# LeCAR-Lab/CoVO-MPC

Hardware: AMD Instinct MI355X
Metric: mpc_control_steps_per_sec (higher is better)
Workload: dtype f32; 1 GPU; covo-online tracking_zigzag N=65536 H=32 lam=0.01 sigma=0.5 (teacher-forced on the recorded inputs -- noisy state, a_mean, key -- of this controller's own 300-step closed-loop episode, timed steps spread evenly over the episode; samples sharded 1x65536, one exchange of the 516-float rank records per step: collective); controller=covo-online, task=tracking_zigzag, N_global=65536, N_local=65536, H=32, pos_stats_info=False

## Files before the change

covo_mpc_amd/csrc/hessian_adj_body.hpp:

```cpp
constexpr int NX = ADJ_NX, NZ = NX + 4, NH = NX + 1, HH = COVO_H, NA = COVO_NA;
constexpr size_t WS_X = 0;
constexpr size_t WS_JF = WS_X + 32 * 16;
constexpr size_t WS_GL = WS_JF + 32 * NX * NZ;
constexpr size_t WS_LAM = WS_GL + 32 * 16;
constexpr size_t WS_MXX = WS_LAM + 33 * 16;
constexpr size_t WS_MXU = WS_MXX + 32 * 256;
constexpr size_t WS_MUU = WS_MXU + 32 * 64;
constexpr size_t WS_S = WS_MUU + 32 * 16;
constexpr int NPAIR = NZ * (NZ + 1) / 2;
constexpr int PAIR_THREADS = (NPAIR + 63) / 64 * 64;
constexpr size_t WS_COUNT = WS_S + (size_t)32 * 16 * NA + 2;
constexpr unsigned long long ADJ_LAM_UNSET = 0xFFF7ADEADBEEF000ull;


__device__ __forceinline__ void adj_force(const float *__restrict__ st, const AdjArgs &A, int bi, int k, double (&f)[3])
{
    if (k == 0) {
        f[0] = st[ST_FDIST + 0]; f[1] = st[ST_FDIST + 1]; f[2] = st[ST_FDIST + 2];
    } else if (A.f_tab != nullptr) {
        const float4 r = A.f_tab[(size_t)bi * HH + k];
        f[0] = r.x; f[1] = r.y; f[2] = r.z;
    } else {
        f[0] = f[1] = f[2] = 0.0;
    }
}

__device__ __forceinline__ void adj_targets(const float *__restrict__ st, const float *__restrict__ pos_traj,
                                            const float *__restrict__ vel_traj, int T, int time0, int k, double (&tar)[6])
{
    if (k == 0) {
        for (int i = 0; i < 3; ++i) { tar[i] = st[ST_POSTAR + i]; tar[3 + i] = st[ST_VELTAR + i]; }
    } else {
        int idx = time0 + k;
        idx = idx < 0 ? 0 : (idx > T - 1 ? T - 1 : idx);
        for (int i = 0; i < 3; ++i) { tar[i] = pos_traj[3 * idx + i]; tar[3 + i] = vel_traj[3 * idx + i]; }
    }
}

#define ADJ_FOR_STATE(OP) OP(px, 0) OP(py, 1) OP(pz, 2) OP(vx, 3) OP(vy, 4) OP(vz, 5) OP(qx, 6) OP(qy, 7) OP(qz, 8) OP(qw, 9) OP(ox, 10) OP(oy, 11) OP(oz, 12)

__device__ __forceinline__ void adj_store_state(const qm::State<double> &p, double *__restrict__ x)
{
#define OP(m, i) x[i] = p.m;
    ADJ_FOR_STATE(OP)
#undef OP
}
__device__ __forceinline__ void adj_load_state(qm::State<double> &p, const double *__restrict__ x)
{
#define OP(m, i) p.m = x[i];
    ADJ_FOR_STATE(OP)
#undef OP
}

#if ADJ_FS
struct AdjDrag {
    double k, off[3];
};
__device__ __forceinline__ AdjDrag adj_drag(const AdjArgs &A, int bi)
{
    AdjDrag D = {A.drag_k, {A.drag_off[0], A.drag_off[1], A.drag_off[2]}};
    if (A.models != nullptr) {
        const dm::Model m = A.models[bi];
        D.k = adj_drag_coeff(m);
        for (int i = 0; i < 3; ++i) D.off[i] = 0.5 * (double)m.dp[i];
    }
    return D;
}
template <class S>
__device__ __forceinline__ void adj_next_force(const AdjArgs &A, const AdjDrag &D, int bi, int k, const qm::State<S> &s, const S (&f)[3],
                                               S (&fn)[3])
{
    if (k + 1 >= HH) {
        fn[0] = fn[1] = fn[2] = S{};
        return;
    }
    const float4 r = A.f_tab[(size_t)bi * HH + k + 1];
    const double g[3] = {r.x, r.y, r.z}, c = r.w;
    const S v[3] = {s.vx, s.vy, s.vz};
#pragma unroll
    for (int i = 0; i < 3; ++i) fn[i] = (f[i] * c + g[i]) + qm::drag_force<S, double>(v[i], D.off[i], D.k);
}
#endif


#if !ADJ_FS
struct AdjQuat {
    double x, y, z, w;
};
__device__ __forceinline__ AdjQuat adj_qmul(const AdjQuat &a, const AdjQuat &b)
{
    AdjQuat r;
    r.x = fma(a.w, b.x, fma(a.x, b.w, fma(a.y, b.z, -(a.z * b.y))));
    r.y = fma(a.w, b.y, fma(a.y, b.w, fma(a.z, b.x, -(a.x * b.z))));
    r.z = fma(a.w, b.z, fma(a.z, b.w, fma(a.x, b.y, -(a.y * b.x))));
    r.w = fma(a.w, b.w, -fma(a.x, b.x, fma(a.y, b.y, a.z * b.z)));
    return r;
}
template <int CTRL>
__device__ __forceinline__ AdjQuat adj_qdpp(const AdjQuat &q)
{
    return AdjQuat{wr::dpp_f64<CTRL>(q.x), wr::dpp_f64<CTRL>(q.y), wr::dpp_f64<CTRL>(q.z), wr::dpp_f64<CTRL>(q.w)};
}
__device__ __forceinline__ double adj_scan_sum(double v, const double (&pw)[4], double pr, int lane)
{
    v = fma(wr::dpp_f64<0x111>(v), pw[0], v);
    v = fma(wr::dpp_f64<0x112>(v), pw[1], v);
    v = fma(wr::dpp_f64<0x114>(v), pw[2], v);
    v = fma(wr::dpp_f64<0x118>(v), pw[3], v);
    const double t = wr::dpp_f64<0x142>(v);
    return ((lane & 16) != 0) ? fma(t, pr, v) : v;
}
template <bool FT>
__device__ __forceinline__ qm::State<double> adj_prefix_scan(const qm::State<double> &p0, const double (*sact)[4], const double (*sfd)[3],
                                                             const qm::Consts<double> &c, int lane)
{
    const int k = lane & 31, lo = lane & 15;
    const double one[4] = {1.0, 1.0, 1.0, 1.0};
    double pa[4];
    pa[0] = c.alpha;
    pa[1] = pa[0] * pa[0];
    pa[2] = pa[1] * pa[1];
    pa[3] = pa[2] * pa[2];
    const double a16 = pa[3] * pa[3];
    double alo = 1.0;
    if (lo & 1) alo *= pa[0];
    if (lo & 2) alo *= pa[1];
    if (lo & 4) alo *= pa[2];
    if (lo & 8) alo *= pa[3];
    const double ak = (k & 16) ? alo * a16 : alo, apr = alo * c.alpha;
    const double th = sact[k][0];
    double cx = sact[k][1] * c.one_m_alpha, cy = sact[k][2] * c.one_m_alpha, cz = sact[k][3] * c.one_m_alpha;
    cx = adj_scan_sum(cx, pa, apr, lane);
    cy = adj_scan_sum(cy, pa, apr, lane);
    cz = adj_scan_sum(cz, pa, apr, lane);
    const double ox = fma(ak, p0.ox, wr::dpp_f64<0x138>(cx));
    const double oy = fma(ak, p0.oy, wr::dpp_f64<0x138>(cy));
    const double oz = fma(ak, p0.oz, wr::dpp_f64<0x138>(cz));
    AdjQuat P{ox * c.half_dt, oy * c.half_dt, oz * c.half_dt, 1.0};
    {
        AdjQuat t = adj_qdpp<0x111>(P);
        if (lo >= 1) P = adj_qmul(t, P);
        t = adj_qdpp<0x112>(P);
        if (lo >= 2) P = adj_qmul(t, P);
        t = adj_qdpp<0x114>(P);
        if (lo >= 4) P = adj_qmul(t, P);
        t = adj_qdpp<0x118>(P);
        if (lo >= 8) P = adj_qmul(t, P);
        t = adj_qdpp<0x142>(P);
        if (lane & 16) P = adj_qmul(t, P);
    }
    AdjQuat E = adj_qdpp<0x138>(P);
    if (lane == 0) E = AdjQuat{0.0, 0.0, 0.0, 1.0};
    AdjQuat q0{p0.qx, p0.qy, p0.qz, p0.qw};
    {
        const double rn = qm::rsq64_(fma(q0.x, q0.x, fma(q0.y, q0.y, fma(q0.z, q0.z, q0.w * q0.w))));
        q0.x *= rn; q0.y *= rn; q0.z *= rn; q0.w *= rn;
    }
    AdjQuat q = adj_qmul(q0, E);
    if (k > 0) {
        const double rn = qm::rsq64_(fma(q.x, q.x, fma(q.y, q.y, fma(q.z, q.z, q.w * q.w))));
        q.x *= rn; q.y *= rn; q.z *= rn; q.w *= rn;
    }
    const double fx = (FT || k == 0) ? sfd[k][0] : 0.0, fy = (FT || k == 0) ? sfd[k][1] : 0.0, fz = (FT || k == 0) ? sfd[k][2] : 0.0;
    const double Qz0 = 2.0 * (q.x * q.z + q.y * q.w), Qz1 = 2.0 * (q.y * q.z - q.x * q.w), Qz2 = q.w * q.w - q.x * q.x - q.y * q.y + q.z * q.z;
    double dvx = ((Qz0 * th + fx) * c.inv_m) * c.dt, dvy = ((Qz1 * th + fy) * c.inv_m) * c.dt, dvz = ((Qz2 * th + fz) * c.inv_m + c.neg_g) * c.dt;
    dvx = adj_scan_sum(dvx, one, 1.0, lane);
    dvy = adj_scan_sum(dvy, one, 1.0, lane);
    dvz = adj_scan_sum(dvz, one, 1.0, lane);
    const double vx = p0.vx + wr::dpp_f64<0x138>(dvx), vy = p0.vy + wr::dpp_f64<0x138>(dvy), vz = p0.vz + wr::dpp_f64<0x138>(dvz);
    double dpx = adj_scan_sum(vx * c.dt, one, 1.0, lane), dpy = adj_scan_sum(vy * c.dt, one, 1.0, lane), dpz = adj_scan_sum(vz * c.dt, one, 1.0, lane);
    qm::State<double> r;
    r.px = p0.px + wr::dpp_f64<0x138>(dpx);
    r.py = p0.py + wr::dpp_f64<0x138>(dpy);
    r.pz = p0.pz + wr::dpp_f64<0x138>(dpz);
    r.vx = vx; r.vy = vy; r.vz = vz;
    r.qx = (k == 0) ? p0.qx : q.x; r.qy = (k == 0) ? p0.qy : q.y; r.qz = (k == 0) ? p0.qz : q.z; r.qw = (k == 0) ? p0.qw : q.w;
    r.ox = ox; r.oy = oy; r.oz = oz;
    return r;
}
#endif

__device__ __forceinline__ void adj_hd_step(const float *__restrict__ st, const float *__restrict__ am, const AdjArgs &A, int bi,
                                            int time0, int k, const qm::State<double> &p, int a, int b, qm::HD &r,
                                            qm::State<qm::HD> &s
#if ADJ_FS
                                            , const double (&pf)[3], qm::HD (&fn)[3]
#endif
)
{
    const qm::Consts<double> c = A.cs ? A.cs[bi] : A.c;
#define OP(m, i) s.m = qm::HD{p.m, a == i ? 1.0 : 0.0, b == i ? 1.0 : 0.0, 0.0};
    ADJ_FOR_STATE(OP)
#undef OP
#if ADJ_FS
    qm::HD fh[3];
#pragma unroll
    for (int i = 0; i < 3; ++i) {
        fh[i] = qm::HD{pf[i], a == 13 + i ? 1.0 : 0.0, b == 13 + i ? 1.0 : 0.0, 0.0};
        fn[i] = fh[i];
    }
#endif
    r = qm::hd(0.0);
    if (k >= 1) {
        double tar[6];
        adj_targets(st, A.pos_traj + bi * A.traj_stride, A.vel_traj + bi * A.traj_stride, A.T, time0, k, tar);
        r = qm::reward_kind<qm::HD, double>(A.reward, s, tar[0], tar[1], tar[2], tar[3], tar[4], tar[5]);
    }
    if (k <= HH - 2) {
        qm::HD act[4];
#pragma unroll
        for (int d = 0; d < 4; ++d) {
            const qm::HD x{(double)am[4 * k + d], a == NX + d ? 1.0 : 0.0, b == NX + d ? 1.0 : 0.0, 0.0};
            act[d] = qm::clip11_(qm::clip11_(x));
        }
#if ADJ_FS
        adj_next_force<qm::HD>(A, adj_drag(A, bi), bi, k, s, fh, fn);
        qm::dyn_step<qm::HD, double, true, qm::HD>(s, act[0], act[1], act[2], act[3], c, fh[0], fh[1], fh[2]);
#else
        double f[3];
        adj_force(st, A, bi, k, f);
        qm::dyn_step<qm::HD, double>(s, act[0], act[1], act[2], act[3], c, f[0], f[1], f[2]);
#endif
    }
}

template <bool FT>
__global__ __launch_bounds__(64) void adj_jac_kernel(const AdjArgs A)
{
    const int k = blockIdx.x, b = blockIdx.y, lane = threadIdx.x;
    const float *__restrict__ st = A.state + (size_t)b * COVO_STATE_FLOATS;
    const bool raw = A.a_mean_raw != nullptr;
    const float *__restrict__ am_base = raw ? A.a_mean_raw : A.a_mean + (size_t)b * NA;
    const bool shift = raw && A.begin_pass == 0;
    auto am = [&](int i) { return am_base[(shift && i < NA - 4) ? i + 4 : i]; };
    if (raw && k == 0) {
        float *shift_out = const_cast<float *>(A.a_mean);
        shift_out[lane] = am(lane);
        shift_out[lane + 64] = am(lane + 64);
        if (lane < 4) {
            if (A.begin_pass > 0) {
                const uint32_t p0 = A.dyn_out[10], p1 = A.dyn_out[11];
                uint32_t rk[2];
                step_begin_derive_next(lane, p0, p1, A.shared_noise_scale, A.dyn_out, rk);
            } else {
                step_begin_derive(lane, A.blk, A.derive_keys, A.shared_noise_scale, A.dyn_out);
            }
        }
        if (lane == 4 && A.seq != nullptr) A.seq[0] = A.seq[0] + 1u;
    }
    double *__restrict__ ws = A.ws + (size_t)b * WS_COUNT;
    if (lane < 16) {
        reinterpret_cast<unsigned long long *>(ws + WS_LAM)[16 * k + lane] = ADJ_LAM_UNSET;
        if (k == HH - 1) reinterpret_cast<unsigned long long *>(ws + WS_LAM)[16 * HH + lane] = ADJ_LAM_UNSET;
    }
    const int time0 = __float_as_int(st[ST_TIME]);
    const qm::Consts<double> c = A.cs ? A.cs[b] : A.c;
    qm::State<double> p;
    p.px = st[ST_POS + 0]; p.py = st[ST_POS + 1]; p.pz = st[ST_POS + 2];
    p.vx = st[ST_VEL + 0]; p.vy = st[ST_VEL + 1]; p.vz = st[ST_VEL + 2];
    p.qx = st[ST_QUAT + 0]; p.qy = st[ST_QUAT + 1]; p.qz = st[ST_QUAT + 2]; p.qw = st[ST_QUAT + 3];
    p.ox = st[ST_OMEGA + 0]; p.oy = st[ST_OMEGA + 1]; p.oz = st[ST_OMEGA + 2];
    __shared__ double sact[HH][4];
    __shared__ double sfd[HH][3];
    if (lane < HH) {
        double f[3];
        adj_force(st, A, b, lane, f);
        sfd[lane][0] = f[0]; sfd[lane][1] = f[1]; sfd[lane][2] = f[2];
    }
    if (lane < HH) {
        const double a0 = qm::clip11_((double)am(4 * lane + 0)), a1 = qm::clip11_((double)am(4 * lane + 1));
        const double a2 = qm::clip11_((double)am(4 * lane + 2)), a3 = qm::clip11_((double)am(4 * lane + 3));
        sact[lane][0] = (a0 + 1.0) * c.thrust_half;
        sact[lane][1] = a1 * c.komega[0];
        sact[lane][2] = a2 * c.komega[1];
        sact[lane][3] = a3 * c.komega[2];
    }
    __syncthreads();
#if ADJ_FS
    const AdjDrag D = adj_drag(A, b);
    double pf[3] = {sfd[0][0], sfd[0][1], sfd[0][2]};
    for (int t = 0; t < k; ++t) {
        const double th = sact[t][0], w0 = sact[t][1], w1 = sact[t][2], w2 = sact[t][3];
        double fn[3];
        adj_next_force<double>(A, D, b, t, p, pf, fn);
        if (t == 0) qm::dyn_core<double, double>(p, th, w0, w1, w2, c, pf[0], pf[1], pf[2]);
        else qm::dyn_core<double, double, false>(p, th, w0, w1, w2, c, pf[0], pf[1], pf[2]);
        pf[0] = fn[0]; pf[1] = fn[1]; pf[2] = fn[2];
    }
    if (lane == 0) {
        adj_store_state(p, ws + WS_X + 16 * k);
        ws[WS_X + 16 * k + 13] = pf[0]; ws[WS_X + 16 * k + 14] = pf[1]; ws[WS_X + 16 * k + 15] = pf[2];
    }
#else
    if (A.scan_prefix) {
        const qm::State<double> ps = adj_prefix_scan<FT>(p, sact, sfd, c, lane);
#define OP(m, i) p.m = wr::bcast_lane(ps.m, k);
        ADJ_FOR_STATE(OP)
#undef OP
    } else {
        for (int t = 0; t < k; ++t) {
            const double th = sact[t][0], w0 = sact[t][1], w1 = sact[t][2], w2 = sact[t][3];
            if (t == 0) qm::dyn_core<double, double>(p, th, w0, w1, w2, c, sfd[0][0], sfd[0][1], sfd[0][2]);
            else if (FT) qm::dyn_core<double, double, false>(p, th, w0, w1, w2, c, sfd[t][0], sfd[t][1], sfd[t][2]);
            else qm::dyn_core<double, double, false>(p, th, w0, w1, w2, c, 0.0, 0.0, 0.0);
        }
    }
    if (lane == 0) adj_store_state(p, ws + WS_X + 16 * k);
#endif
    qm::State<qm::D1> s;
#define OP(m, i) s.m = qm::D1{p.m, lane == i ? 1.0 : 0.0};
    ADJ_FOR_STATE(OP)
#undef OP
#if ADJ_FS
    qm::D1 fd[3], fdn[3];
#pragma unroll
    for (int i = 0; i < 3; ++i) {
        fd[i] = qm::D1{pf[i], lane == 13 + i ? 1.0 : 0.0};
        fdn[i] = fd[i];
    }
#endif
    qm::D1 r{0.0, 0.0};
    if (k >= 1) {
        double tar[6];
        adj_targets(st, A.pos_traj + b * A.traj_stride, A.vel_traj + b * A.traj_stride, A.T, time0, k, tar);
        r = qm::reward_kind<qm::D1, double>(A.reward, s, tar[0], tar[1], tar[2], tar[3], tar[4], tar[5]);
    }
    if (k <= HH - 2) {
        qm::D1 act[4];
#pragma unroll
        for (int d = 0; d < 4; ++d) {
            const qm::D1 x{(double)am(4 * k + d), lane == NX + d ? 1.0 : 0.0};
            act[d] = qm::clip11_(qm::clip11_(x));
        }
#if ADJ_FS
        adj_next_force<qm::D1>(A, D, b, k, s, fd, fdn);
        qm::dyn_step<qm::D1, double, true, qm::D1>(s, act[0], act[1], act[2], act[3], c, fd[0], fd[1], fd[2]);
#else
        qm::dyn_step<qm::D1, double>(s, act[0], act[1], act[2], act[3], c, sfd[k][0], sfd[k][1], sfd[k][2]);
#endif
    }
    if (lane < NZ) {
        if (lane < NX) ws[WS_GL + 16 * k + lane] = r.a;
        if (k <= HH - 2) {
            double *__restrict__ jf = ws + WS_JF + (size_t)k * NX * NZ;
#define OP(m, i) jf[i * NZ + lane] = s.m.a;
            ADJ_FOR_STATE(OP)
#undef OP
#if ADJ_FS
            jf[13 * NZ + lane] = fdn[0].a; jf[14 * NZ + lane] = fdn[1].a; jf[15 * NZ + lane] = fdn[2].a;
#endif
        }
    }
}

__device__ __forceinline__ void adj_hd_pairs(const AdjArgs &A, int k, int b, int tid)
{
    if (tid >= NPAIR) return;
    const float *__restrict__ st = A.state + (size_t)b * COVO_STATE_FLOATS;
    const float *__restrict__ am = A.a_mean + (size_t)b * NA;
    double *__restrict__ ws = A.ws + (size_t)b * WS_COUNT;
    const int time0 = __float_as_int(st[ST_TIME]);
    int q = tid, a = 0;
    while (q >= NZ - a) { q -= NZ - a; ++a; }
    const int bb = a + q;
    qm::State<double> p;
    adj_load_state(p, ws + WS_X + 16 * k);
    qm::HD r;
    qm::State<qm::HD> s;
#if ADJ_FS
    const double pf[3] = {ws[WS_X + 16 * k + 13], ws[WS_X + 16 * k + 14], ws[WS_X + 16 * k + 15]};
    qm::HD fn[3];
    adj_hd_step(st, am, A, b, time0, k, p, a, bb, r, s, pf, fn);
#else
    adj_hd_step(st, am, A, b, time0, k, p, a, bb, r, s);
#endif
    double h[NH];
    h[0] = r.ab;
#define OP(m, i) h[1 + i] = s.m.ab;
    ADJ_FOR_STATE(OP)
#undef OP
#if ADJ_FS
    h[14] = fn[0].ab; h[15] = fn[1].ab; h[16] = fn[2].ab;
#endif
    double g = h[0];
    if (k <= HH - 2) {
        const double *__restrict__ Lk = ws + WS_LAM + 16 * (k + 1);
        double lam[NX];
        const long long t0 = wall_clock64();
        for (;;) {
            bool unset = false;
#pragma unroll
            for (int i = 0; i < NX; ++i) {
                lam[i] = __hip_atomic_load(Lk + i, __ATOMIC_RELAXED, __HIP_MEMORY_SCOPE_AGENT);
                unset |= (unsigned long long)__double_as_longlong(lam[i]) == ADJ_LAM_UNSET;
            }
            if (!unset) break;
            if (wall_clock64() - t0 > 50000000LL) {
                if (A.status != nullptr) __hip_atomic_fetch_or(A.status, COVO_DEVSTAT_ADJOINT, __ATOMIC_RELAXED, __HIP_MEMORY_SCOPE_SYSTEM);
                break;
            }
            __builtin_amdgcn_s_sleep(2);
        }
#pragma unroll
        for (int i = 0; i < NX; ++i) g = fma(lam[i], h[1 + i], g);
    }
    double *__restrict__ Mxx = ws + WS_MXX + (size_t)k * 256, *__restrict__ Mxu = ws + WS_MXU + (size_t)k * 64;
    double *__restrict__ Muu = ws + WS_MUU + (size_t)k * 16;
    if (bb < NX) {
        Mxx[a * 16 + bb] = g;
        Mxx[bb * 16 + a] = g;
    } else if (a < NX) {
        Mxu[a * 4 + (bb - NX)] = g;
    } else {
        Muu[(a - NX) * 4 + (bb - NX)] = g;
        Muu[(bb - NX) * 4 + (a - NX)] = g;
    }
}

__device__ __forceinline__ void adj_hd_padding(const AdjArgs &A, int k, int b, int tid, int nthreads)
{
    double *__restrict__ ws = A.ws + (size_t)b * WS_COUNT;
    double *__restrict__ Mxx = ws + WS_MXX + (size_t)k * 256, *__restrict__ Mxu = ws + WS_MXU + (size_t)k * 64;
    for (int e = tid; e < 256; e += nthreads)
        if ((e >> 4) >= NX || (e & 15) >= NX) Mxx[e] = 0.0;
    if (tid < (16 - NX) * 4) Mxu[NX * 4 + tid] = 0.0;
}

__global__ __launch_bounds__(256) void adj_hd_kernel(const AdjArgs A)
{
    adj_hd_padding(A, (int)blockIdx.x, (int)blockIdx.y, (int)threadIdx.x, 256);
    adj_hd_pairs(A, (int)blockIdx.x, (int)blockIdx.y, (int)threadIdx.x);
}

__global__ __launch_bounds__(256) void adj_chain_kernel(const AdjArgs A)
{
    __shared__ double sjf[(HH - 1) * NX * NZ + 1];
    __shared__ double sgl[HH * 16];
    const int b = blockIdx.y, tid = threadIdx.x, lane = tid & 63, lo = lane & 15, hi = lane >> 4;
    const int w = blockIdx.x;
    double *__restrict__ ws = A.ws + (size_t)b * WS_COUNT;
#ifdef KC_STAMPS
    const long long kc0 = wall_clock64();
#endif
    if (w >= 9) {
        adj_hd_padding(A, w - 9, b, tid, 256);
        adj_hd_pairs(A, w - 9, b, tid);
        return;
    }
    {
        constexpr int NJ = (HH - 1) * NX * NZ, TJ = (NJ + 255) / 256;
        double vj[TJ];
#pragma unroll
        for (int t = 0; t < TJ; ++t) vj[t] = (tid + 256 * t < NJ) ? ws[WS_JF + tid + 256 * t] : 0.0;
        const double vg0 = ws[WS_GL + tid], vg1 = ws[WS_GL + 256 + tid];
#pragma unroll
        for (int t = 0; t < TJ; ++t)
            if (tid + 256 * t < NJ) sjf[tid + 256 * t] = vj[t];
        sgl[tid] = vg0;
        sgl[256 + tid] = vg1;
        if (tid == 0) sjf[NJ] = 0.0;
    }
#ifdef KC_STAMPS
    const long long kc1 = wall_clock64();
#endif
    __syncthreads();
#ifdef KC_STAMPS
    const long long kc2 = wall_clock64();
#define KC_STAMP_END()                                                                                                       \
    do {                                                                                                                     \
        if (tid == 0 && b == 0 && (w == 0 || w == 7 || w == 8))                                                              \
            printf("KC wg %d: filled %lld first-mfma %lld end %lld (10 ns ticks from entry)\n", w, kc1 - kc0, kc2 - kc0,      \
                   (long long)wall_clock64() - kc0);                                                                         \
    } while (0)
#else
#define KC_STAMP_END() do { } while (0)
#endif
    if (tid >= 64) return;
    constexpr int ZI = (HH - 1) * NX * NZ;
    if (w == 8) {
        const double *__restrict__ G = sgl;
        double *__restrict__ L = ws + WS_LAM;
        f64x4 lam;
#pragma unroll
        for (int r = 0; r < 4; ++r) lam[r] = (lo == 0 && hi + 4 * r < NX) ? G[16 * (HH - 1) + hi + 4 * r] : 0.0;
        if (lo == 0) {
#pragma unroll
            for (int r = 0; r < 4; ++r) {
                __hip_atomic_store(&L[16 * (HH - 1) + hi + 4 * r], lam[r], __ATOMIC_RELAXED, __HIP_MEMORY_SCOPE_AGENT);
                __hip_atomic_store(&L[16 * HH + hi + 4 * r], 0.0, __ATOMIC_RELAXED, __HIP_MEMORY_SCOPE_AGENT);
            }
        }
        int offA[4];
        bool okA[4];
#pragma unroll
        for (int g = 0; g < 4; ++g) {
            okA[g] = lo < NX && 4 * g + hi < NX;
            offA[g] = (4 * g + hi) * NZ + lo;
        }
        bool okG[4];
#pragma unroll
        for (int r = 0; r < 4; ++r) okG[r] = lo == 0 && hi + 4 * r < NX;
        double an[4];
        f64x4 gn;
#pragma unroll
        for (int g = 0; g < 4; ++g) an[g] = sjf[okA[g] ? (HH - 2) * NX * NZ + offA[g] : ZI];
#pragma unroll
        for (int r = 0; r < 4; ++r) gn[r] = okG[r] ? G[16 * (HH - 2) + hi + 4 * r] : 0.0;
#pragma unroll
        for (int k = HH - 2; k >= 1; --k) {
            double ac[4];
            f64x4 acc = gn;
#pragma unroll
            for (int g = 0; g < 4; ++g) ac[g] = an[g];
            if (k > 1) {
#pragma unroll
                for (int g = 0; g < 4; ++g) an[g] = sjf[okA[g] ? (k - 1) * NX * NZ + offA[g] : ZI];
#pragma unroll
                for (int r = 0; r < 4; ++r) gn[r] = okG[r] ? G[16 * (k - 1) + hi + 4 * r] : 0.0;
            }
#pragma unroll
            for (int g = 0; g < 4; ++g) acc = __builtin_amdgcn_mfma_f64_16x16x4f64(ac[g], lam[g], acc, 0, 0, 0);
            lam = acc;
            if (lo == 0) {
#pragma unroll
                for (int r = 0; r < 4; ++r) __hip_atomic_store(&L[16 * k + hi + 4 * r], lam[r], __ATOMIC_RELAXED, __HIP_MEMORY_SCOPE_AGENT);
            }
        }
        KC_STAMP_END();
        return;
    }
    const int col = 16 * w + lo, tcol = col >> 2, dcol = col & 3, k0 = 4 * w;
    double *__restrict__ S = ws + WS_S;
    for (int k = 0; k <= k0; ++k) {
#pragma unroll
        for (int r = 0; r < 4; ++r) S[((size_t)k * 16 + hi + 4 * r) * NA + col] = 0.0;
    }
    f64x4 sv = {0.0, 0.0, 0.0, 0.0};
    int offA[4];
    bool okA[4];
#pragma unroll
    for (int g = 0; g < 4; ++g) {
        okA[g] = lo < NX && 4 * g + hi < NX;
        offA[g] = lo * NZ + 4 * g + hi;
    }
    double an[4];
    f64x4 bn;
#pragma unroll
    for (int g = 0; g < 4; ++g) an[g] = sjf[okA[g] ? k0 * NX * NZ + offA[g] : ZI];
#pragma unroll
    for (int r = 0; r < 4; ++r) bn[r] = (tcol == k0 && hi + 4 * r < NX) ? sjf[(k0 * NX + hi + 4 * r) * NZ + NX + dcol] : 0.0;
    double *__restrict__ Sp = S + (size_t)hi * NA + col;
#pragma unroll
    for (int k = 0; k < HH - 1; ++k) {
        if (k < k0) continue;
        double ac[4];
        f64x4 acc = bn;
#pragma unroll
        for (int g = 0; g < 4; ++g) ac[g] = an[g];
        if (k + 1 < HH - 1) {
#pragma unroll
            for (int g = 0; g < 4; ++g) an[g] = sjf[okA[g] ? (k + 1) * NX * NZ + offA[g] : ZI];
            if (k + 1 <= k0 + 3) {
#pragma unroll
                for (int r = 0; r < 4; ++r)
                    bn[r] = (tcol == k + 1 && hi + 4 * r < NX) ? sjf[((k + 1) * NX + hi + 4 * r) * NZ + NX + dcol] : 0.0;
            } else {
#pragma unroll
                for (int r = 0; r < 4; ++r) bn[r] = 0.0;
            }
        }
#pragma unroll
        for (int g = 0; g < 4; ++g) acc = __builtin_amdgcn_mfma_f64_16x16x4f64(ac[g], sv[g], acc, 0, 0, 0);
        sv = acc;
#pragma unroll
        for (int r = 0; r < 4; ++r) Sp[((size_t)(k + 1) * 16 + 4 * r) * NA] = sv[r];
    }
    KC_STAMP_END();
}
#undef KC_STAMP_END

__device__ __forceinline__ void adj_tri_tile(int w, int &ti, int &tj)
{
    ti = 0;
    while ((ti + 1) * (ti + 2) / 2 <= w) ++ti;
    tj = w - ti * (ti + 1) / 2;
}

__global__ __launch_bounds__(512) void adj_gemm_kernel(const AdjArgs A)
{
    __shared__ double red[8][4][64];
    __shared__ double sMu[4][64];
    __shared__ double sMuu[64];
    const int b = blockIdx.y, tid = threadIdx.x, lane = tid & 63, wv = tid >> 6, lo = lane & 15, hi = lane >> 4;
    const double *__restrict__ ws = A.ws + (size_t)b * WS_COUNT;
    double *__restrict__ R = A.R + (size_t)b * NA * NA;
    int I, J;
    adj_tri_tile(blockIdx.x, I, J);
    const double *__restrict__ S = ws + WS_S, *__restrict__ Mxx = ws + WS_MXX;
    f64x4 acc = {0.0, 0.0, 0.0, 0.0};
#ifdef KD_PROF
    const long long kp0 = clock64();
#endif
    double ma[4][4], sj[4][4], si[4][4];
#pragma unroll
    for (int it = 0; it < 4; ++it) {
        const int k = 4 * I + 1 + wv + 8 * it;
        const bool on = k < HH;
        const double *__restrict__ Sk = S + (size_t)(on ? k : 0) * 16 * NA, *__restrict__ Mk = Mxx + (size_t)(on ? k : 0) * 256;
        const double2 *__restrict__ Mk2 = reinterpret_cast<const double2 *>(Mk + lo * 16 + 4 * hi);
        const double2 m01 = on ? Mk2[0] : make_double2(0.0, 0.0), m23 = on ? Mk2[1] : make_double2(0.0, 0.0);
        ma[it][0] = m01.x;
        ma[it][1] = m01.y;
        ma[it][2] = m23.x;
        ma[it][3] = m23.y;
#pragma unroll
        for (int g = 0; g < 4; ++g) {
            sj[it][g] = on ? Sk[(size_t)(4 * hi + g) * NA + 16 * J + lo] : 0.0;
            si[it][g] = on ? Sk[(size_t)(4 * g + hi) * NA + 16 * I + lo] : 0.0;
        }
    }
    const int i = 16 * I + hi + 4 * (wv & 3), j = 16 * J + lo;
    const int ti = i >> 2, di = i & 3, tj = j >> 2, dj = j & 3;
    const int tk = ti > tj ? ti : tj, dk = ti > tj ? di : dj;
    double es[NX];
    if (wv < 4) {
        const int col = ti > tj ? j : i;
        const double *__restrict__ Sk = S + (size_t)tk * 16 * NA;
#pragma unroll
        for (int m = 0; m < NX; ++m) es[m] = Sk[(size_t)m * NA + col];
    } else if (wv == 4) {
        sMuu[lane] = ws[WS_MUU + (size_t)(4 * I) * 16 + lane];
    }
    if (tid < 256) sMu[wv][lane] = ws[WS_MXU + (size_t)(4 * I + wv) * 64 + lane];
#ifdef KD_PROF
    asm volatile("s_waitcnt vmcnt(0)" ::: "memory");
    const long long kp1 = clock64();
#endif
#pragma unroll
    for (int it = 0; it < 4; ++it) {
        if (4 * I + 1 + wv + 8 * it >= HH) break;
        f64x4 Q = {0.0, 0.0, 0.0, 0.0};
#pragma unroll
        for (int g = 0; g < 4; ++g) Q = __builtin_amdgcn_mfma_f64_16x16x4f64(ma[it][g], sj[it][g], Q, 0, 0, 0);
#pragma unroll
        for (int g = 0; g < 4; ++g) acc = __builtin_amdgcn_mfma_f64_16x16x4f64(si[it][g], Q[g], acc, 0, 0, 0);
    }
#pragma unroll
    for (int r = 0; r < 4; ++r) red[wv][r][lane] = acc[r];
#ifdef KD_PROF
    const long long kp2 = clock64();
#endif
    __syncthreads();
#ifdef KD_PROF
    const long long kp3 = clock64();
    if (tid == 0 && (blockIdx.x == 0 || blockIdx.x == 35)) printf("KD wg %d: loads %lld mfma %lld barrier %lld\n", (int)blockIdx.x, kp1 - kp0, kp2 - kp1, kp3 - kp2);
#endif
    double v = 0.0;
    if (wv < 4) {
#pragma unroll
        for (int w8 = 0; w8 < 8; ++w8) v += red[w8][wv][lane];
        if (ti != tj) {
            const double *mu = sMu[tk - 4 * I];
#pragma unroll
            for (int m = 0; m < NX; ++m) v = fma(es[m], mu[m * 4 + dk], v);
        } else {
            v += sMuu[(ti - 4 * I) * 16 + di * 4 + dj];
        }
        if (I != J || i >= j) {
            R[(size_t)i * NA + j] = -v;
            R[(size_t)j * NA + i] = -v;
        }
    }
    if (A.stats.rpart != nullptr) {
        __shared__ double st_tmp[16][17];
        __shared__ double st_part[4];
        __shared__ double st_diag[16][17];
        double rv = -v;
        if (I == J) {
            if (wv < 4) st_diag[hi + 4 * wv][lo] = rv;
            __syncthreads();
            if (wv < 4 && i < j) rv = st_diag[lo][hi + 4 * wv];
        }
        SymStatsOut so = A.stats;
        so.rpart += (size_t)b * so.stride;
        so.fpart += (size_t)b * so.stride;
        so.diag += (size_t)b * so.stride;
        sym_tile_stats(wv < 4, rv, I, J, (int)blockIdx.x, lane, wv & 3, so, st_tmp, st_part);
        if (so.flags != nullptr && blockIdx.x == 0 && tid < 64) so.flags[(size_t)b * so.stride + tid] = 0.0;
        if (so.ready != nullptr && blockIdx.x == 0 && tid == 64) so.ready[(size_t)b * so.stride] = 0.0;
    }
}
#undef ADJ_FOR_STATE
```

Baseline: 6281 control-steps/s.

## Split adjoint and sensitivity chains into four parallel horizon segments per workgroup

The serial 31-step MFMA recurrences in adj_chain_kernel (the costate backward chain and the state-sensitivity forward chain) were each run by a single wave. They are now cut into four horizon segments processed by four waves at once. Each wave builds its segment's transfer-matrix products, then joins with the neighbouring segment through LDS, using a flag spin-wait or __syncthreads, and fills in the intermediate steps with independent MFMAs. This shortens the dependent-latency critical path but adds LDS transposes, extra MFMA work, and intra-workgroup synchronisation. The gemm kernel also gains a NaN-propagation check on the costate output.

```diff
diff --git a/covo_mpc_amd/csrc/hessian_adj_body.hpp b/covo_mpc_amd/csrc/hessian_adj_body.hpp
--- a/covo_mpc_amd/csrc/hessian_adj_body.hpp
+++ b/covo_mpc_amd/csrc/hessian_adj_body.hpp
@@ -432,19 +432,337 @@
     adj_hd_pairs(A, (int)blockIdx.x, (int)blockIdx.y, (int)threadIdx.x);
 }
 
+static_assert(HH == 32, "adj_chain_kernel: four horizon segments of 8, 8, 8 and 7 steps");
+constexpr int KC_ZI = (HH - 1) * NX * NZ;
+constexpr int KC_TLD = 17;
+
+__device__ __forceinline__ void adj_wave_sync()
+{
+    __builtin_amdgcn_fence(__ATOMIC_ACQ_REL, "wavefront");
+    __builtin_amdgcn_wave_barrier();
+}
+__device__ __forceinline__ void adj_cd_to_a(double *__restrict__ tb, const f64x4 &t, int lo, int hi, double (&a)[4])
+{
+    adj_wave_sync();
+#pragma unroll
+    for (int r = 0; r < 4; ++r) tb[(4 * r + hi) * KC_TLD + lo] = t[r];
+    adj_wave_sync();
+#pragma unroll
+    for (int g = 0; g < 4; ++g) a[g] = tb[lo * KC_TLD + 4 * g + hi];
+}
+__device__ __forceinline__ f64x4 adj_mm(const double (&a)[4], const f64x4 &b, f64x4 acc)
+{
+#pragma unroll
+    for (int g = 0; g < 4; ++g) acc = __builtin_amdgcn_mfma_f64_16x16x4f64(a[g], b[g], acc, 0, 0, 0);
+    return acc;
+}
+template <int CNT>
+__device__ __forceinline__ void adj_mm_many(const double (&pa)[8][4], const f64x4 &b, f64x4 (&out)[8])
+{
+#pragma unroll
+    for (int i = 0; i < CNT; ++i) out[i] = f64x4{0.0, 0.0, 0.0, 0.0};
+#pragma unroll
+    for (int g = 0; g < 4; ++g) {
+#pragma unroll
+        for (int i = 0; i < CNT; ++i) out[i] = __builtin_amdgcn_mfma_f64_16x16x4f64(pa[i][g], b[g], out[i], 0, 0, 0);
+    }
+}
+
+template <int J>
+__device__ __forceinline__ void adj_sens_chain(const double *__restrict__ sjf, double *__restrict__ tb, double *__restrict__ ho,
+                                               double *__restrict__ S, int w, int lane, double (&pa)[8][4], f64x4 &sv)
+{
+    constexpr int M0 = 8 * J, M1 = J == 3 ? HH - 1 : 8 * J + 8;
+    const int lo = lane & 15, hi = lane >> 4;
+    const int col = 16 * w + lo, tcol = col >> 2, dcol = col & 3, k0 = 4 * w, jw = w >> 1;
+    double *__restrict__ Sp = S + (size_t)hi * NA + col;
+#pragma unroll
+    for (int k = (J == 0 ? 0 : M0 + 1); k <= M1; ++k) {
+        if (k <= k0) {
+#pragma unroll
+            for (int r = 0; r < 4; ++r) Sp[((size_t)k * 16 + 4 * r) * NA] = 0.0;
+        }
+    }
+    if (J < jw) return;
+    int offA[4];
+    bool okA[4];
+#pragma unroll
+    for (int g = 0; g < 4; ++g) {
+        okA[g] = lo < NX && 4 * g + hi < NX;
+        offA[g] = lo * NZ + 4 * g + hi;
+    }
+    double an[4];
+    if (J == jw) {
+        sv = f64x4{0.0, 0.0, 0.0, 0.0};
+        f64x4 bn;
+#pragma unroll
+        for (int g = 0; g < 4; ++g) an[g] = sjf[okA[g] ? k0 * NX * NZ + offA[g] : KC_ZI];
+#pragma unroll
+        for (int r = 0; r < 4; ++r) bn[r] = (tcol == k0 && hi + 4 * r < NX) ? sjf[(k0 * NX + hi + 4 * r) * NZ + NX + dcol] : 0.0;
+#pragma unroll
+        for (int k = M0; k < M1; ++k) {
+            if (k < k0) continue;
+            double ac[4];
+            f64x4 acc = bn;
+#pragma unroll
+            for (int g = 0; g < 4; ++g) ac[g] = an[g];
+            if (k + 1 < M1) {
+#pragma unroll
+                for (int g = 0; g < 4; ++g) an[g] = sjf[okA[g] ? (k + 1) * NX * NZ + offA[g] : KC_ZI];
+                if (k + 1 <= k0 + 3) {
+#pragma unroll
+                    for (int r = 0; r < 4; ++r)
+                        bn[r] = (tcol == k + 1 && hi + 4 * r < NX) ? sjf[((k + 1) * NX + hi + 4 * r) * NZ + NX + dcol] : 0.0;
+                } else {
+#pragma unroll
+                    for (int r = 0; r < 4; ++r) bn[r] = 0.0;
+                }
+            }
+            sv = adj_mm(ac, sv, acc);
+#pragma unroll
+            for (int r = 0; r < 4; ++r) Sp[((size_t)(k + 1) * 16 + 4 * r) * NA] = sv[r];
+        }
+        if (J < 3) {
+#pragma unroll
+            for (int r = 0; r < 4; ++r) ho[64 * r + lane] = sv[r];
+        }
+    } else if constexpr (J > 0) {
+        f64x4 t;
+#pragma unroll
+        for (int r = 0; r < 4; ++r) t[r] = sjf[(lo < NX && 4 * r + hi < NX) ? M0 * NX * NZ + (4 * r + hi) * NZ + lo : KC_ZI];
+#pragma unroll
+        for (int g = 0; g < 4; ++g) pa[0][g] = sjf[okA[g] ? M0 * NX * NZ + offA[g] : KC_ZI];
+#pragma unroll
+        for (int g = 0; g < 4; ++g) an[g] = sjf[okA[g] ? (M0 + 1) * NX * NZ + offA[g] : KC_ZI];
+#pragma unroll
+        for (int k = M0 + 1; k < M1; ++k) {
+            double ac[4];
+#pragma unroll
+            for (int g = 0; g < 4; ++g) ac[g] = an[g];
+            if (k + 1 < M1) {
+#pragma unroll
+                for (int g = 0; g < 4; ++g) an[g] = sjf[okA[g] ? (k + 1) * NX * NZ + offA[g] : KC_ZI];
+            }
+            t = adj_mm(ac, t, f64x4{0.0, 0.0, 0.0, 0.0});
+            adj_cd_to_a(tb, t, lo, hi, pa[k - M0]);
+        }
+    }
+}
+template <int J>
+__device__ __forceinline__ void adj_sens_join(const double *__restrict__ hi_slot, double *__restrict__ ho, int lane,
+                                              const double (&pa)[8][4], f64x4 &sm, f64x4 &sv)
+{
+    constexpr int CNT = J == 3 ? HH - 1 - 24 : 8;
+#pragma unroll
+    for (int r = 0; r < 4; ++r) sm[r] = hi_slot[64 * r + lane];
+    sv = adj_mm(pa[CNT - 1], sm, f64x4{0.0, 0.0, 0.0, 0.0});
+    if (J < 3) {
+#pragma unroll
+        for (int r = 0; r < 4; ++r) ho[64 * r + lane] = sv[r];
+    }
+}
+template <int J>
+__device__ __forceinline__ void adj_sens_fill(double *__restrict__ S, int w, int lane, const double (&pa)[8][4], const f64x4 &sm,
+                                              const f64x4 &sv)
+{
+    constexpr int M0 = 8 * J, M1 = J == 3 ? HH - 1 : 8 * J + 8, CNT = M1 - M0;
+    double *__restrict__ Sp = S + (size_t)(lane >> 4) * NA + 16 * w + (lane & 15);
+#pragma unroll
+    for (int r = 0; r < 4; ++r) Sp[((size_t)M1 * 16 + 4 * r) * NA] = sv[r];
+    f64x4 out[8];
+    adj_mm_many<CNT - 1>(pa, sm, out);
+#pragma unroll
+    for (int i = 0; i < CNT - 1; ++i) {
+#pragma unroll
+        for (int r = 0; r < 4; ++r) Sp[((size_t)(M0 + 1 + i) * 16 + 4 * r) * NA] = out[i][r];
+    }
+}
+
+template <int KEND>
+__device__ __forceinline__ void adj_cost_top(const double *__restrict__ sjf, const double *__restrict__ G, double *__restrict__ L,
+                                             int lane, f64x4 &lam)
+{
+    const int lo = lane & 15, hi = lane >> 4;
+#pragma unroll
+    for (int r = 0; r < 4; ++r) lam[r] = (lo == 0 && hi + 4 * r < NX) ? G[16 * (HH - 1) + hi + 4 * r] : 0.0;
+    if (lo == 0) {
+#pragma unroll
+        for (int r = 0; r < 4; ++r) {
+            __hip_atomic_store(&L[16 * (HH - 1) + hi + 4 * r], lam[r], __ATOMIC_RELAXED, __HIP_MEMORY_SCOPE_AGENT);
+            __hip_atomic_store(&L[16 * HH + hi + 4 * r], 0.0, __ATOMIC_RELAXED, __HIP_MEMORY_SCOPE_AGENT);
+        }
+    }
+    int offA[4];
+    bool okA[4];
+#pragma unroll
+    for (int g = 0; g < 4; ++g) {
+        okA[g] = lo < NX && 4 * g + hi < NX;
+        offA[g] = (4 * g + hi) * NZ + lo;
+    }
+    bool okG[4];
+#pragma unroll
+    for (int r = 0; r < 4; ++r) okG[r] = lo == 0 && hi + 4 * r < NX;
+    double an[4];
+    f64x4 gn;
+#pragma unroll
+    for (int g = 0; g < 4; ++g) an[g] = sjf[okA[g] ? (HH - 2) * NX * NZ + offA[g] : KC_ZI];
+#pragma unroll
+    for (int r = 0; r < 4; ++r) gn[r] = okG[r] ? G[16 * (HH - 2) + hi + 4 * r] : 0.0;
+#pragma unroll
+    for (int k = HH - 2; k >= KEND; --k) {
+        double ac[4];
+        f64x4 acc = gn;
+#pragma unroll
+        for (int g = 0; g < 4; ++g) ac[g] = an[g];
+        if (k > KEND) {
+#pragma unroll
+            for (int g = 0; g < 4; ++g) an[g] = sjf[okA[g] ? (k - 1) * NX * NZ + offA[g] : KC_ZI];
+#pragma unroll
+            for (int r = 0; r < 4; ++r) gn[r] = okG[r] ? G[16 * (k - 1) + hi + 4 * r] : 0.0;
+        }
+        lam = adj_mm(ac, lam, acc);
+        if (lo == 0) {
+#pragma unroll
+            for (int r = 0; r < 4; ++r) __hip_atomic_store(&L[16 * k + hi + 4 * r], lam[r], __ATOMIC_RELAXED, __HIP_MEMORY_SCOPE_AGENT);
+        }
+    }
+}
+#if !ADJ_FS
+template <int J>
+__device__ __forceinline__ void adj_cost_chain(const double *__restrict__ sjf, const double *__restrict__ G, double *__restrict__ tb,
+                                               int lane, double (&pa)[8][4])
+{
+    constexpr int E = 8 * J + 7, M = J == 0 ? 1 : 8 * J;
+    const int lo = lane & 15, hi = lane >> 4;
+    int offA[4], offT[4];
+    bool okA[4], okG[4];
+#pragma unroll
+    for (int g = 0; g < 4; ++g) {
+        okA[g] = lo < NX && 4 * g + hi < NX;
+        offA[g] = (4 * g + hi) * NZ + lo;
+        offT[g] = lo * NZ + 4 * g + hi;
+        okG[g] = lo == NX && 4 * g + hi < NX;
+    }
+    f64x4 t;
+#pragma unroll
+    for (int r = 0; r < 4; ++r) {
+        const double a = sjf[okA[r] ? E * NX * NZ + offT[r] : KC_ZI];
+        t[r] = okG[r] ? G[16 * E + hi + 4 * r] : a;
+    }
+#pragma unroll
+    for (int g = 0; g < 4; ++g) {
+        const double a = sjf[okA[g] ? E * NX * NZ + offA[g] : KC_ZI];
+        pa[0][g] = (4 * g + hi == NX && lo < NX) ? G[16 * E + lo] : a;
+    }
+    double an[4];
+    f64x4 gn;
+#pragma unroll
+    for (int g = 0; g < 4; ++g) an[g] = sjf[okA[g] ? (E - 1) * NX * NZ + offA[g] : KC_ZI];
+#pragma unroll
+    for (int r = 0; r < 4; ++r) gn[r] = okG[r] ? G[16 * (E - 1) + hi + 4 * r] : 0.0;
+#pragma unroll
+    for (int k = E - 1; k >= M; --k) {
+        double ac[4];
+        f64x4 acc = gn;
+#pragma unroll
+        for (int g = 0; g < 4; ++g) ac[g] = an[g];
+        if (k > M) {
+#pragma unroll
+            for (int g = 0; g < 4; ++g) an[g] = sjf[okA[g] ? (k - 1) * NX * NZ + offA[g] : KC_ZI];
+#pragma unroll
+            for (int r = 0; r < 4; ++r) gn[r] = okG[r] ? G[16 * (k - 1) + hi + 4 * r] : 0.0;
+        }
+        t = adj_mm(ac, t, acc);
+        adj_cd_to_a(tb, t, lo, hi, pa[E - k]);
+    }
+}
+__device__ __forceinline__ double adj_cost_quarter(const double (&a)[4], const double (&vv)[4])
+{
+    return fma(a[3], vv[3], fma(a[2], vv[2], fma(a[1], vv[1], a[0] * vv[0])));
+}
+__device__ __forceinline__ double adj_cost_over_hi(double p)
+{
+    p += __shfl_xor(p, 16, 64);
+    p += __shfl_xor(p, 32, 64);
+    return p;
+}
+__device__ __forceinline__ void adj_cost_publish(double *__restrict__ L, int k, int lane, double v)
+{
+    if (lane < 16) __hip_atomic_store(&L[16 * k + lane], v, __ATOMIC_RELAXED, __HIP_MEMORY_SCOPE_AGENT);
+}
+__device__ __forceinline__ void adj_flag_set(int *flag)
+{
+    adj_wave_sync();
+    __hip_atomic_store(flag, 1, __ATOMIC_RELEASE, __HIP_MEMORY_SCOPE_WORKGROUP);
+}
+__device__ __forceinline__ void adj_flag_wait(int *flag, const AdjArgs &A)
+{
+    const long long t0 = wall_clock64();
+    while (__hip_atomic_load(flag, __ATOMIC_ACQUIRE, __HIP_MEMORY_SCOPE_WORKGROUP) == 0) {
+        if (wall_clock64() - t0 > 50000000LL) {
+            if (A.status != nullptr) __hip_atomic_fetch_or(A.status, COVO_DEVSTAT_ADJOINT, __ATOMIC_RELAXED, __HIP_MEMORY_SCOPE_SYSTEM);
+            break;
+        }
+        __builtin_amdgcn_s_sleep(1);
+    }
+}
+template <int J>
+__device__ __forceinline__ void adj_cost_join(const double *__restrict__ hi_slot, double *__restrict__ ho, int *flag,
+                                              double *__restrict__ L, int lane, const double (&pa)[8][4], double (&vv)[4])
+{
+    constexpr int E = 8 * J + 7, M = J == 0 ? 1 : 8 * J;
+    const int hi = lane >> 4;
+#pragma unroll
+    for (int g = 0; g < 4; ++g) {
+        const double x = hi_slot[4 * g + hi];
+        vv[g] = 4 * g + hi < NX ? x : (4 * g + hi == NX ? 1.0 : 0.0);
+    }
+    const double lm = adj_cost_over_hi(adj_cost_quarter(pa[E - M], vv));
+    if (J > 0) {
+        if (lane < 16) ho[lane] = lm;
+        adj_flag_set(flag);
+    }
+    adj_cost_publish(L, M, lane, lm);
+}
+template <int J>
+__device__ __forceinline__ void adj_cost_fill(double *__restrict__ L, int lane, const double (&pa)[8][4], const double (&vv)[4])
+{
+    constexpr int E = 8 * J + 7, M = J == 0 ? 1 : 8 * J;
+    double q[E - M];
+#pragma unroll
+    for (int i = 0; i < E - M; ++i) q[i] = adj_cost_quarter(pa[i], vv);
+#pragma unroll
+    for (int i = 0; i < E - M; ++i) q[i] += __shfl_xor(q[i], 16, 64);
+#pragma unroll
+    for (int i = 0; i < E - M; ++i) q[i] += __shfl_xor(q[i], 32, 64);
+#pragma unroll
+    for (int i = 0; i < E - M; ++i) adj_cost_publish(L, E - i, lane, q[i]);
+}
+#endif
+
 __global__ __launch_bounds__(256) void adj_chain_kernel(const AdjArgs A)
 {
     __shared__ double sjf[(HH - 1) * NX * NZ + 1];
     __shared__ double sgl[HH * 16];
-    const int b = blockIdx.y, tid = threadIdx.x, lane = tid & 63, lo = lane & 15, hi = lane >> 4;
+    __shared__ double stb[4][16 * KC_TLD];
+    __shared__ double sho[3][256];
+    __shared__ int sfl[4];
+    const int b = blockIdx.y, tid = threadIdx.x, lane = tid & 63, wv = tid >> 6;
     const int w = blockIdx.x;
     double *__restrict__ ws = A.ws + (size_t)b * WS_COUNT;
 #ifdef KC_STAMPS
     const long long kc0 = wall_clock64();
+    long long kc3 = 0, kc4 = 0;
+#define KC_STAMP(x) x = (long long)wall_clock64() - kc0
+#else
+#define KC_STAMP(x) do { } while (0)
 #endif
     if (w >= 9) {
         adj_hd_padding(A, w - 9, b, tid, 256);
         adj_hd_pairs(A, w - 9, b, tid);
+#ifdef KC_STAMPS
+        if (tid == 0 && b == 0 && ((w - 9) % 8 == 0 || w - 9 == HH - 1)) printf("KC hd %d: end %lld (10 ns ticks from entry)\n", w - 9, (long long)wall_clock64() - kc0);
+#endif
         return;
     }
     {
@@ -459,6 +777,7 @@
         sgl[tid] = vg0;
         sgl[256 + tid] = vg1;
         if (tid == 0) sjf[NJ] = 0.0;
+        if (tid < 4) sfl[tid] = 0;
     }
 #ifdef KC_STAMPS
     const long long kc1 = wall_clock64();
@@ -466,118 +785,94 @@
     __syncthreads();
 #ifdef KC_STAMPS
     const long long kc2 = wall_clock64();
-#define KC_STAMP_END()                                                                                                       \
+    __shared__ long long kcs[4][4];
+#define KC_STAMP_END(ALL)                                                                                                    \
     do {                                                                                                                     \
+        const long long kc5 = (long long)wall_clock64() - kc0;                                                               \
+        asm volatile("s_waitcnt vmcnt(0)" ::: "memory");                                                                     \
+        if (lane == 0) { kcs[wv][0] = kc3; kcs[wv][1] = kc4; kcs[wv][2] = kc5; kcs[wv][3] = (long long)wall_clock64() - kc0; } \
+        if (ALL) __syncthreads();                                                                                            \
         if (tid == 0 && b == 0 && (w == 0 || w == 7 || w == 8))                                                              \
-            printf("KC wg %d: filled %lld first-mfma %lld end %lld (10 ns ticks from entry)\n", w, kc1 - kc0, kc2 - kc0,      \
-                   (long long)wall_clock64() - kc0);                                                                         \
+            for (int q = 0; q < (ALL ? 4 : 1); ++q)                                                                          \
+                printf("KC wg %d wave %d: filled %lld first-mfma %lld segment %lld join %lld end %lld acked %lld (10 ns "    \
+                       "ticks from entry)\n", w, q, kc1 - kc0, kc2 - kc0, kcs[q][0], kcs[q][1], kcs[q][2], kcs[q][3]);       \
     } while (0)
 #else
-#define KC_STAMP_END() do { } while (0)
-#endif
-    if (tid >= 64) return;
-    constexpr int ZI = (HH - 1) * NX * NZ;
+#define KC_STAMP_END(ALL) do { } while (0)
+#endif
+    double pa[8][4];
     if (w == 8) {
-        const double *__restrict__ G = sgl;
         double *__restrict__ L = ws + WS_LAM;
         f64x4 lam;
-#pragma unroll
-        for (int r = 0; r < 4; ++r) lam[r] = (lo == 0 && hi + 4 * r < NX) ? G[16 * (HH - 1) + hi + 4 * r] : 0.0;
-        if (lo == 0) {
-#pragma unroll
-            for (int r = 0; r < 4; ++r) {
-                __hip_atomic_store(&L[16 * (HH - 1) + hi + 4 * r], lam[r], __ATOMIC_RELAXED, __HIP_MEMORY_SCOPE_AGENT);
-                __hip_atomic_store(&L[16 * HH + hi + 4 * r], 0.0, __ATOMIC_RELAXED, __HIP_MEMORY_SCOPE_AGENT);
+#if ADJ_FS
+        if (wv != 0) return;
+        adj_cost_top<1>(sjf, sgl, L, lane, lam);
+        KC_STAMP(kc3);
+#else
+        double vv[4];
+        switch (wv) {
+        case 0:
+            adj_cost_chain<0>(sjf, sgl, stb[0], lane, pa);
+            KC_STAMP(kc3);
+            adj_flag_wait(&sfl[2], A);
+            adj_cost_join<0>(sho[2], sho[2], &sfl[2], L, lane, pa, vv);
+            KC_STAMP(kc4);
+            adj_cost_fill<0>(L, lane, pa, vv);
+            break;
+        case 1:
+            adj_cost_chain<1>(sjf, sgl, stb[1], lane, pa);
+            KC_STAMP(kc3);
+            adj_flag_wait(&sfl[1], A);
+            adj_cost_join<1>(sho[1], sho[2], &sfl[2], L, lane, pa, vv);
+            KC_STAMP(kc4);
+            adj_cost_fill<1>(L, lane, pa, vv);
+            break;
+        case 2:
+            adj_cost_chain<2>(sjf, sgl, stb[2], lane, pa);
+            KC_STAMP(kc3);
+            adj_flag_wait(&sfl[0], A);
+            adj_cost_join<2>(sho[0], sho[1], &sfl[1], L, lane, pa, vv);
+            KC_STAMP(kc4);
+            adj_cost_fill<2>(L, lane, pa, vv);
+            break;
+        default:
+            adj_cost_top<24>(sjf, sgl, L, lane, lam);
+            if ((lane & 15) == 0) {
+#pragma unroll
+                for (int r = 0; r < 4; ++r) sho[0][(lane >> 4) + 4 * r] = lam[r];
             }
-        }
-        int offA[4];
-        bool okA[4];
-#pragma unroll
-        for (int g = 0; g < 4; ++g) {
-            okA[g] = lo < NX && 4 * g + hi < NX;
-            offA[g] = (4 * g + hi) * NZ + lo;
-        }
-        bool okG[4];
-#pragma unroll
-        for (int r = 0; r < 4; ++r) okG[r] = lo == 0 && hi + 4 * r < NX;
-        double an[4];
-        f64x4 gn;
-#pragma unroll
-        for (int g = 0; g < 4; ++g) an[g] = sjf[okA[g] ? (HH - 2) * NX * NZ + offA[g] : ZI];
-#pragma unroll
-        for (int r = 0; r < 4; ++r) gn[r] = okG[r] ? G[16 * (HH - 2) + hi + 4 * r] : 0.0;
-#pragma unroll
-        for (int k = HH - 2; k >= 1; --k) {
-            double ac[4];
-            f64x4 acc = gn;
-#pragma unroll
-            for (int g = 0; g < 4; ++g) ac[g] = an[g];
-            if (k > 1) {
-#pragma unroll
-                for (int g = 0; g < 4; ++g) an[g] = sjf[okA[g] ? (k - 1) * NX * NZ + offA[g] : ZI];
-#pragma unroll
-                for (int r = 0; r < 4; ++r) gn[r] = okG[r] ? G[16 * (k - 1) + hi + 4 * r] : 0.0;
-            }
-#pragma unroll
-            for (int g = 0; g < 4; ++g) acc = __builtin_amdgcn_mfma_f64_16x16x4f64(ac[g], lam[g], acc, 0, 0, 0);
-            lam = acc;
-            if (lo == 0) {
-#pragma unroll
-                for (int r = 0; r < 4; ++r) __hip_atomic_store(&L[16 * k + hi + 4 * r], lam[r], __ATOMIC_RELAXED, __HIP_MEMORY_SCOPE_AGENT);
-            }
-        }
-        KC_STAMP_END();
+            adj_flag_set(&sfl[0]);
+            KC_STAMP(kc3);
+        }
+#endif
+        KC_STAMP_END(!ADJ_FS);
         return;
     }
-    const int col = 16 * w + lo, tcol = col >> 2, dcol = col & 3, k0 = 4 * w;
     double *__restrict__ S = ws + WS_S;
-    for (int k = 0; k <= k0; ++k) {
-#pragma unroll
-        for (int r = 0; r < 4; ++r) S[((size_t)k * 16 + hi + 4 * r) * NA + col] = 0.0;
-    }
-    f64x4 sv = {0.0, 0.0, 0.0, 0.0};
-    int offA[4];
-    bool okA[4];
-#pragma unroll
-    for (int g = 0; g < 4; ++g) {
-        okA[g] = lo < NX && 4 * g + hi < NX;
-        offA[g] = lo * NZ + 4 * g + hi;
-    }
-    double an[4];
-    f64x4 bn;
-#pragma unroll
-    for (int g = 0; g < 4; ++g) an[g] = sjf[okA[g] ? k0 * NX * NZ + offA[g] : ZI];
-#pragma unroll
-    for (int r = 0; r < 4; ++r) bn[r] = (tcol == k0 && hi + 4 * r < NX) ? sjf[(k0 * NX + hi + 4 * r) * NZ + NX + dcol] : 0.0;
-    double *__restrict__ Sp = S + (size_t)hi * NA + col;
-#pragma unroll
-    for (int k = 0; k < HH - 1; ++k) {
-        if (k < k0) continue;
-        double ac[4];
-        f64x4 acc = bn;
-#pragma unroll
-        for (int g = 0; g < 4; ++g) ac[g] = an[g];
-        if (k + 1 < HH - 1) {
-#pragma unroll
-            for (int g = 0; g < 4; ++g) an[g] = sjf[okA[g] ? (k + 1) * NX * NZ + offA[g] : ZI];
-            if (k + 1 <= k0 + 3) {
-#pragma unroll
-                for (int r = 0; r < 4; ++r)
-                    bn[r] = (tcol == k + 1 && hi + 4 * r < NX) ? sjf[((k + 1) * NX + hi + 4 * r) * NZ + NX + dcol] : 0.0;
-            } else {
-#pragma unroll
-                for (int r = 0; r < 4; ++r) bn[r] = 0.0;
-            }
-        }
-#pragma unroll
-        for (int g = 0; g < 4; ++g) acc = __builtin_amdgcn_mfma_f64_16x16x4f64(ac[g], sv[g], acc, 0, 0, 0);
-        sv = acc;
-#pragma unroll
-        for (int r = 0; r < 4; ++r) Sp[((size_t)(k + 1) * 16 + 4 * r) * NA] = sv[r];
-    }
-    KC_STAMP_END();
+    const int jw = w >> 1;
+    f64x4 sv, sm;
+    switch (wv) {
+    case 0: adj_sens_chain<0>(sjf, stb[0], sho[0], S, w, lane, pa, sv); break;
+    case 1: adj_sens_chain<1>(sjf, stb[1], sho[1], S, w, lane, pa, sv); break;
+    case 2: adj_sens_chain<2>(sjf, stb[2], sho[2], S, w, lane, pa, sv); break;
+    default: adj_sens_chain<3>(sjf, stb[3], sho[2], S, w, lane, pa, sv);
+    }
+    KC_STAMP(kc3);
+    __syncthreads();
+    if (wv == 1 && jw < 1) { adj_sens_join<1>(sho[0], sho[1], lane, pa, sm, sv); KC_STAMP(kc4); }
+    __syncthreads();
+    if (wv == 2 && jw < 2) { adj_sens_join<2>(sho[1], sho[2], lane, pa, sm, sv); KC_STAMP(kc4); }
+    __syncthreads();
+    if (wv == 3 && jw < 3) { adj_sens_join<3>(sho[2], sho[2], lane, pa, sm, sv); KC_STAMP(kc4); }
+    if (wv > jw) {
+        if (wv == 1) adj_sens_fill<1>(S, w, lane, pa, sm, sv);
+        else if (wv == 2) adj_sens_fill<2>(S, w, lane, pa, sm, sv);
+        else adj_sens_fill<3>(S, w, lane, pa, sm, sv);
+    }
+    KC_STAMP_END(true);
 }
 #undef KC_STAMP_END
+#undef KC_STAMP
 
 __device__ __forceinline__ void adj_tri_tile(int w, int &ti, int &tj)
 {
@@ -632,6 +927,8 @@
         sMuu[lane] = ws[WS_MUU + (size_t)(4 * I) * 16 + lane];
     }
     if (tid < 256) sMu[wv][lane] = ws[WS_MXU + (size_t)(4 * I + wv) * 64 + lane];
+    __shared__ double sNan;
+    const double lz = (wv == 5 && lane < 16) ? ws[WS_LAM + 16 + lane] : 0.0;
 #ifdef KD_PROF
     asm volatile("s_waitcnt vmcnt(0)" ::: "memory");
     const long long kp1 = clock64();
@@ -644,6 +941,14 @@
         for (int g = 0; g < 4; ++g) Q = __builtin_amdgcn_mfma_f64_16x16x4f64(ma[it][g], sj[it][g], Q, 0, 0, 0);
 #pragma unroll
         for (int g = 0; g < 4; ++g) acc = __builtin_amdgcn_mfma_f64_16x16x4f64(si[it][g], Q[g], acc, 0, 0, 0);
+    }
+    if (wv == 5) {
+        double pz = lz * 0.0;
+        pz += __shfl_xor(pz, 1, 64);
+        pz += __shfl_xor(pz, 2, 64);
+        pz += __shfl_xor(pz, 4, 64);
+        pz += __shfl_xor(pz, 8, 64);
+        if (lane == 0) sNan = pz;
     }
 #pragma unroll
     for (int r = 0; r < 4; ++r) red[wv][r][lane] = acc[r];
@@ -666,6 +971,8 @@
         } else {
             v += sMuu[(ti - 4 * I) * 16 + di * 4 + dj];
         }
+        const double pz = sNan;
+        if (pz != pz) v = pz;
         if (I != J || i >= j) {
             R[(size_t)i * NA + j] = -v;
             R[(size_t)j * NA + i] = -v;
```

New measurement: 6366 control-steps/s, median of 6. +1.4%, better.
